# ODD2/DFD-CLIP

Hardware: AMD Instinct MI355X
Metric: 1-sec clips/sec (30x224x224 frames) ViT-B/16 (higher is better)
Workload: dtype bf16

## Files before the change

dfd-clip_amd/capi.py:

```python
import ctypes
import os
from ctypes import POINTER, Structure, c_char_p, c_double, c_float, c_int, c_int32, c_int64, c_size_t, c_uint32, c_void_p

import torch

PKG_DIR = os.path.dirname(os.path.abspath(__file__))
LIB_PATH = os.path.join(PKG_DIR, "libdfdclip_hip.so")

F32, BF16 = 0, 1
EPI_BIAS, EPI_BIAS_QUICKGELU, EPI_BIAS_RESIDUAL, EPI_PATCH_EMBED, EPI_QKV_EXPORT, EPI_RESIDUAL_POS, EPI_BIAS_GELU = range(7)
ABI_VERSION = 17

_DTYPE = {torch.float32: F32, torch.bfloat16: BF16}
FP8 = 2
FP8_MAX = 448.0
FP8_MIN_ROWS = 1024


class DfdError(RuntimeError):
    pass


GEMM_STREAM_OUT = 1
GEMM_SPARE_IF_FREE = 2
GEMM_C_BLOCKED = 4
GEMM_A_BLOCKED = 8


class GemmExtra(Structure):
    _fields_ = [("pos", c_void_p), ("cls", c_void_p), ("k_export", c_void_p), ("v_export", c_void_p),
                ("tokens", c_int32), ("frames_per_clip", c_int32), ("residual", c_void_p), ("qkv_first", c_int32),
                ("drop_rng", c_void_p), ("drop_site", c_uint32), ("drop_p", c_float), ("flags", c_uint32)]


OPTIM_SGD, OPTIM_ADAMW = 0, 1


class OptimExtra(Structure):
    _fields_ = [("kind", c_int32), ("reserved", c_int32), ("beta1", c_double), ("beta2", c_double), ("eps", c_double),
                ("step", c_int64), ("exp_avg_sq", c_void_p)]


class DropoutDesc(Structure):
    _fields_ = [("rng_state", c_void_p), ("site", c_uint32), ("p", c_float)]


class Dropout:
    __slots__ = ("rng", "site", "p")

    def __init__(self, rng, site, p):
        assert rng.is_cuda and rng.dtype == torch.int64 and rng.numel() == 2 and 0.0 <= p < 1.0
        self.rng, self.site, self.p = rng, int(site), float(p)

    def desc(self):
        return DropoutDesc(self.rng.data_ptr(), self.site, self.p)


def _drop(d):
    return ctypes.byref(d.desc()) if d is not None and d.p > 0 else None
# ... 227 lines not shown
    s3 = (c_float * 3)(*[float(v) for v in std])
    if patch_rows:
        assert out.dim() == 2 and out.shape[0] == n * (res // patch) ** 2
        kpad = out.shape[1]
    else:
        assert tuple(out.shape) == (n, 3, res, res)
        kpad = 0
    _check(load_library().dfd_preprocess_u8(_ptr(frames), n, h, w, res, patch, int(bool(antialias)), m3, s3, _ptr(out),
                                            _DTYPE[out.dtype], 1 if patch_rows else 0, kpad, _stream()), "dfd_preprocess_u8")
    return out


_profile = {"epilogue": None, "events": [], "base": None}


def profile_gemm(epilogue=None):
    _profile["epilogue"] = epilogue
    _profile["events"] = []
    _profile["base"] = None
    if epilogue is not None:
        _profile["base"] = torch.cuda.Event(enable_timing=True)
        _profile["base"].record()


def profile_gemm_collect():
    base = _profile["base"]
    spans = [(base.elapsed_time(a), base.elapsed_time(b), flops) for a, b, flops in _profile["events"]]
    profile_gemm(None)
    return spans


def gemm(a, w, c, bias=None, epilogue=EPI_BIAS, m=None, pos=None, cls=None, k_export=None, v_export=None, tokens=0,
         frames_per_clip=0, residual=None, qkv_first=0, drop=None, stream_out=False, spare_cus=0, tile_blocks=0, spare_if_free=False,
         c_blocked=False, a_blocked=False):
    _dev(a, w, c, bias, pos, cls, k_export, v_export, residual)
    assert a.dtype == w.dtype and a.stride(1) == 1 and w.stride(1) == 1 and c.stride(1) == 1
    M = a.shape[0] if m is None else m
    N, K = w.shape
    assert a.shape[1] == K
    assert residual is None or (residual.dtype == c.dtype and residual.stride(0) == c.stride(0))
    assert drop is None or epilogue == EPI_RESIDUAL_POS
    assert 0 <= epilogue <= EPI_BIAS_GELU, f"unknown epilogue {epilogue}"
    if c_blocked or a_blocked:
        blk = c if c_blocked else a
        assert blk.shape[0] >= (M + 15) // 16 * 16, "a blocked matrix needs its rows rounded up to 16"
    extra = GemmExtra(_ptr(pos).value, _ptr(cls).value, _ptr(k_export).value, _ptr(v_export).value, tokens, frames_per_clip,
                      _ptr(residual).value, qkv_first, drop.rng.data_ptr() if drop is not None and drop.p > 0 else None,
                      drop.site if drop is not None else 0, drop.p if drop is not None else 0.0, (GEMM_STREAM_OUT if stream_out else 0) | (GEMM_SPARE_IF_FREE if spare_if_free else 0) | ((int(spare_cus) & 0xff) << 8) | ((int(tile_blocks) & 0xf) << 16)
                      | (GEMM_C_BLOCKED if c_blocked else 0) | (GEMM_A_BLOCKED if a_blocked else 0))
    timed = _profile["epilogue"] == epilogue
    if timed:
        e0, e1 = torch.cuda.Event(enable_timing=True), torch.cuda.Event(enable_timing=True)
        e0.record()
    _check(load_library().dfd_gemm(_ptr(a), a.stride(0), _ptr(w), w.stride(0), _DTYPE[a.dtype], _ptr(c), c.stride(0),
                                   _DTYPE[c.dtype], _ptr(bias), epilogue, ctypes.byref(extra), M, N, K, _stream()), "dfd_gemm")
    if timed:
        e1.record()
        _profile["events"].append((e0, e1, 2.0 * M * N * K))
    return c


def gemm_fp8(a, w, c, col_scale, bias=None, epilogue=EPI_BIAS, m=None, out_inv_scale=0.0, pos=None, k_export=None, v_export=None,
             tokens=0, frames_per_clip=0, qkv_first=0, stream_out=False, spare_cus=0, spare_if_free=False):
    _dev(a, w, c, col_scale, bias, pos, k_export, v_export)
    assert a.element_size() == 1 and w.element_size() == 1 and a.stride(1) == 1 and w.stride(1) == 1 and c.stride(1) == 1
    assert col_scale.dtype == torch.float32 and col_scale.is_contiguous()
    M = a.shape[0] if m is None else m
    N, K = w.shape
    assert a.shape[1] == K and col_scale.numel() == N
    c_dtype = FP8 if c.element_size() == 1 else _DTYPE[c.dtype]
    extra = GemmExtra(_ptr(pos).value, None, _ptr(k_export).value, _ptr(v_export).value, tokens, frames_per_clip, None, qkv_first,
                      None, 0, 0.0, (GEMM_STREAM_OUT if stream_out else 0) | (GEMM_SPARE_IF_FREE if spare_if_free else 0) | ((int(spare_cus) & 0xff) << 8))
    timed = _profile["epilogue"] == epilogue
    if timed:
        e0, e1 = torch.cuda.Event(enable_timing=True), torch.cuda.Event(enable_timing=True)
        e0.record()
    _check(load_library().dfd_gemm_fp8(_ptr(a), a.stride(0), _ptr(w), w.stride(0), _ptr(c), c.stride(0), c_dtype, _ptr(col_scale),
                                       _ptr(bias), float(out_inv_scale), epilogue, ctypes.byref(extra), M, N, K, _stream()),
           "dfd_gemm_fp8")
    if timed:
        e1.record()
        _profile["events"].append((e0, e1, 2.0 * M * N * K))
# ... 383 lines not shown
```

dfd-clip_amd/csrc/gemm.hip:

```cpp
#include "gemm_args.hpp"
#include "gelu.hpp"
#include "../../include/dfdclip_hooks.h"

namespace {

constexpr int BM = 128, BN = 128;
constexpr int ROW_BYTES = 64;
constexpr int ROW_STRIDE = 80;
constexpr int TILE_BYTES = BM * ROW_STRIDE;
constexpr int EPI_SPLITK_SLAB = 100;

template <typename CT> __device__ __forceinline__ void store_c(void* C, int64_t off, float v) {
  static_cast<CT*>(C)[off] = from_f32<CT>(v);
}

template <typename CT, int EPI>
__device__ __forceinline__ void epilogue_elem(const GemmArgs& a, int64_t m, int n, float acc) {
  if (m >= a.M || n >= a.N) return;
  if constexpr (EPI == DFD_EPI_BIAS) {
    store_c<CT>(a.C, m * a.ldc + n, acc + (a.bias ? a.bias[n] : 0.f));
  } else if constexpr (EPI == DFD_EPI_BIAS_QUICKGELU) {
    store_c<CT>(a.C, m * a.ldc + n, quick_gelu(acc + (a.bias ? a.bias[n] : 0.f)));
  } else if constexpr (EPI == DFD_EPI_BIAS_GELU) {
    store_c<CT>(a.C, m * a.ldc + n, gelu_erf(acc + (a.bias ? a.bias[n] : 0.f)));
// ... 237 lines not shown
}

static int fill_extra(GemmArgs& a, int epilogue, const dfd_gemm_extra* extra, int c_dtype, int64_t ldc, int64_t M, int N) {
  if (epilogue == DFD_EPI_PATCH_EMBED) {
    DFD_REQUIRE(extra && extra->pos && extra->cls && extra->tokens > 1, "dfd_gemm: PATCH_EMBED needs extra.pos, extra.cls, extra.tokens");
    DFD_REQUIRE(M % (extra->tokens - 1) == 0, "dfd_gemm: PATCH_EMBED M=%lld is not a whole number of frames", (long long)M);
    DFD_REQUIRE(c_dtype == DFD_F32 && ldc >= N, "dfd_gemm: PATCH_EMBED writes an f32 token matrix");
  } else {
    DFD_REQUIRE(ldc >= N, "dfd_gemm: ldc=%lld < N", (long long)ldc);
  }
  if (epilogue == DFD_EPI_QKV_EXPORT) {
    DFD_REQUIRE(extra && extra->tokens > 1 && (extra->qkv_first == 0 || extra->qkv_first == 1) && N % (3 - extra->qkv_first) == 0,
                "dfd_gemm: QKV_EXPORT needs extra.tokens, qkv_first in {0, 1} and N a multiple of the column blocks present");
    DFD_REQUIRE(M % extra->tokens == 0, "dfd_gemm: QKV_EXPORT M=%lld is not a whole number of frames", (long long)M);
    DFD_REQUIRE(!extra->k_export == !extra->v_export, "dfd_gemm: QKV_EXPORT needs both k_export and v_export or neither");
    DFD_REQUIRE(!extra->pos || extra->frames_per_clip > 0, "dfd_gemm: QKV_EXPORT with pos needs frames_per_clip");
  }
  if (epilogue == DFD_EPI_RESIDUAL_POS) {
    DFD_REQUIRE(extra && extra->tokens > 1, "dfd_gemm: RESIDUAL_POS needs extra.tokens (patches per frame + 1)");
    DFD_REQUIRE(!extra->pos || extra->frames_per_clip > 0, "dfd_gemm: RESIDUAL_POS with pos needs frames_per_clip");
  }
  if (extra) {
    a.pos = extra->pos; a.cls = extra->cls; a.k_export = extra->k_export; a.v_export = extra->v_export;
    a.residual = epilogue == DFD_EPI_RESIDUAL_POS ? extra->residual : nullptr;
    a.tokens = extra->tokens; a.frames_per_clip = extra->frames_per_clip > 0 ? extra->frames_per_clip : 1;
    a.qkv_first = epilogue == DFD_EPI_QKV_EXPORT ? extra->qkv_first : 0;
    a.stream_out = (extra->flags & DFD_GEMM_STREAM_OUT) ? 1 : 0;
    a.spare_cus = (int)((extra->flags >> DFD_GEMM_SPARE_CUS_SHIFT) & 0xff);
    a.spare_if_free = (extra->flags & DFD_GEMM_SPARE_IF_FREE) ? 1 : 0;
    a.tile_rows = 32 * (int)((extra->flags >> DFD_GEMM_TILE_BLOCKS_SHIFT) & 0xf);
    a.c_blocked = (extra->flags & DFD_GEMM_C_BLOCKED) ? 1 : 0;
    a.a_blocked = (extra->flags & DFD_GEMM_A_BLOCKED) ? 1 : 0;
    a.pair = a.c_blocked | a.a_blocked;
    DFD_REQUIRE(a.tile_rows == 0 || a.tile_rows == 224 || a.tile_rows == 256, "dfd_gemm: tile blocks must be 0, 7 or 8");
    if (epilogue == DFD_EPI_RESIDUAL_POS && extra->drop_rng && extra->drop_p > 0.f) {
      DFD_REQUIRE(extra->drop_p < 1.f, "dfd_gemm: drop_p=%f", (double)extra->drop_p);
      const dfd_dropout_t dd{extra->drop_rng, extra->drop_site, extra->drop_p};
      a.drop = dfd_make_drop(&dd);
    }
  }
  return DFD_OK;
}

static thread_local int g_last_path = 0;
static thread_local int g_gemm_variant = 0;
extern "C" int dfd_gemm_last_path(void) { return g_last_path; }
extern "C" int dfd_gemm_set_variant(int variant) {
  const int old = g_gemm_variant;
  g_gemm_variant = variant;
  return old;
}

static thread_local int g_pair_variant = 0;
static thread_local int64_t g_pair_launches = 0;
extern "C" int dfd_gemm_pair_set_variant(int variant) {
  const int old = g_pair_variant;
  g_pair_variant = variant;
  return old;
}
extern "C" int64_t dfd_gemm_pair_launches(void) { return g_pair_launches; }
extern "C" int dfd_gemm_pair_plan(int64_t M, int D, int H) {
  if (g_pair_variant == 1 || g_gemm_variant == 1 || M < 1 || D < 1 || H < 1) return 0;
  if (M < 1024 && g_pair_variant != 2) return 0;
  void* const any = reinterpret_cast<void*>(uintptr_t{256});
  GemmArgs fc{}, pr{};
  fc.A = pr.A = any; fc.W = pr.W = any; fc.C = pr.C = any;
  fc.M = pr.M = M; fc.pair = pr.pair = 1;
  fc.N = H; fc.K = D; fc.lda = D; fc.ldw = D; fc.ldc = H; fc.c_blocked = 1;
  pr.N = D; pr.K = H; pr.lda = H; pr.ldw = H; pr.ldc = D; pr.a_blocked = 1;
  return dfd_gemm256e_serves(fc, DFD_BF16, DFD_EPI_BIAS_QUICKGELU) && dfd_gemm256e_serves(pr, DFD_BF16, DFD_EPI_BIAS) ? 1 : 0;
}

static int try_persistent_kernels(GemmArgs& a, int c_dtype, int epilogue, bool f8, hipStream_t st, int* path) {
  const int epi_p = epilogue == DFD_EPI_QKV_EXPORT && a.k_export == nullptr ? DFD_EPI_BIAS : epilogue;
  a.no_dynamic = g_gemm_variant != 3;
  if (a.pair) {
    if (g_pair_variant == 1) a.c_blocked = a.a_blocked = 0;
    *path = 257;
    const int rc = f8 || g_gemm_variant == 1 ? 1 : dfd_gemm256e_try(a, c_dtype, epi_p, st);
    if (rc == 1) {
      dfd_set_error("dfd_gemm: DFD_GEMM_C_BLOCKED / DFD_GEMM_A_BLOCKED: the ping-pong kernel does not serve this call (bf16, N %% 256 == 0, "
                    "K %% 128 == 0, K >= 384, ld %% 64 == 0, BIAS_QUICKGELU / BIAS_GELU for C, BIAS for A; got M=%lld N=%d K=%d)",
                    (long long)a.M, a.N, a.K);
      return DFD_ERR_INVALID_ARG;
    }
    if (rc == 0 && (a.c_blocked || a.a_blocked)) ++g_pair_launches;
    return rc;
  }
  int rc = g_gemm_variant == 1 ? 1 : (f8 ? dfd_gemm256e_f8_try : dfd_gemm256e_try)(a, c_dtype, epi_p, st);
  *path = 257;
  if (rc != 1) return rc;
  rc = (f8 ? dfd_gemm256p_f8_try : dfd_gemm256p_try)(a, c_dtype, epi_p, st);
  *path = 256;
  return rc;
}

extern "C" int dfd_gemm(const void* A, int64_t lda, const void* W, int64_t ldw, int ab_dtype, void* C, int64_t ldc,
                        int c_dtype, const float* bias, int epilogue, const dfd_gemm_extra* extra, int64_t M, int N,
                        int K, void* stream) {
  DFD_REQUIRE(A && W && C, "dfd_gemm: null pointer");
  DFD_REQUIRE(M >= 0 && N > 0 && K > 0, "dfd_gemm: bad shape M=%lld N=%d K=%d", (long long)M, N, K);
  DFD_REQUIRE(ab_dtype == DFD_F32 || ab_dtype == DFD_BF16, "dfd_gemm: ab_dtype=%d", ab_dtype);
  DFD_REQUIRE(c_dtype == DFD_F32 || c_dtype == DFD_BF16, "dfd_gemm: c_dtype=%d", c_dtype);
  DFD_REQUIRE(!(ab_dtype == DFD_F32 && c_dtype == DFD_BF16), "dfd_gemm: f32 operands with bf16 output unsupported");
  DFD_REQUIRE(K % 32 == 0, "dfd_gemm: K=%d must be a multiple of 32", K);
  const int esz = ab_dtype == DFD_F32 ? 4 : 2;
  DFD_REQUIRE(lda >= K && ldw >= K && (lda * esz) % 16 == 0 && (ldw * esz) % 16 == 0, "dfd_gemm: lda=%lld ldw=%lld must be >= K and 16-byte multiples", (long long)lda, (long long)ldw);
  DFD_REQUIRE(dfd_aligned16(A) && dfd_aligned16(W), "dfd_gemm: A and W must be 16-byte aligned");
// ... 81 lines not shown
```

dfd-clip_amd/csrc/gemm256e.hip:

```cpp
#include <mutex>
#include <unordered_map>

#include "gemm256p_common.hpp"

namespace {

constexpr int UNIT = 128 * ROWB;
constexpr int DEPTH = 6;
constexpr int NB = 2 * (DEPTH - 1);

template <int EPI, int RB, bool F8, bool CF8, bool ABLK = false>
__global__ __launch_bounds__(512) void gemm256e_kernel(const GemmArgs a, int tiles_m, int tiles_n) {
  static_assert(!F8 || RB == 8, "fp8 form: 256-row tiles only");
  static_assert(!CF8 || (F8 && EPI != DFD_EPI_QKV_EXPORT), "fp8 output: fp8 operands, plain, QuickGELU or GELU epilogue");
  constexpr int ESZ = F8 ? 1 : 2;
  constexpr int TMU = 32 * RB;
  constexpr int WROWS = 16 * RB;
  constexpr int HB = RB - 4;
  constexpr int NCV = F8 ? 2 : 1;
  constexpr int S1 = CF8 ? RB : 2 * RB;
  constexpr int S2 = 4 * RB;
  static_assert(!ABLK || (!F8 && EPI == DFD_EPI_BIAS), "blocked A: bf16 operands, plain epilogue");
  constexpr bool C_BLK = !F8 && (EPI == DFD_EPI_BIAS_QUICKGELU || EPI == DFD_EPI_BIAS_GELU);
  constexpr bool A_BLK = ABLK;
  __shared__ __attribute__((aligned(1024))) unsigned char smem[RING + 8 * STAGE];
  const int tid = threadIdx.x;
  const int lane = tid & 63;
  const int wave = __builtin_amdgcn_readfirstlane(tid >> 6);
  const int wr = wave >> 2, wc = wave & 3;
  const int ntiles = tiles_m * tiles_n;

  const int G = gridDim.x, bid = blockIdx.x;
  const int xcd = bid & 7, q8 = G >> 3, r8 = G & 7;
  const int pos = xcd_position();

  const OperandSrds<F8, CF8, A_BLK, C_BLK> srd(a);
  const __amdgpu_buffer_rsrc_t srdA = srd.A, srdW = srd.W, srdC = srd.C;
  const v4i srdB = words(a.bias ? a.bias : reinterpret_cast<const float*>(a.W), a.bias ? a.N * 4 : 0);
  [[maybe_unused]] const v4i srdS = words(F8 ? a.col_scale : reinterpret_cast<const float*>(a.W), F8 ? a.N * 4 : 0);
  const int cnt_x = q8 + (xcd < r8 ? 1 : 0), off_x = pos - (bid >> 3);
  const v4i srdT = words(reinterpret_cast<const float*>(a.sched ? a.sched : reinterpret_cast<const uint32_t*>(a.W)), a.sched ? 8 * 128 : 0);

  const uint32_t lda2 = (uint32_t)(a.lda * ESZ), ldw2 = (uint32_t)(a.ldw * ESZ);
  const uint32_t a_last = (uint32_t)(a.M - 1) * lda2;
  constexpr bool a_blk = A_BLK;
  constexpr int a_kstep = a_blk ? (int)DFD_BLK_UNIT : ROWB;
  uint32_t vA[2][2], vW[2];
  auto set_a = [&](const Tile& t, int ha) {
    int l = lane;
    asm volatile("" : "+v"(l));
    const uint32_t pr = (uint32_t)(l >> 3), pp = (uint32_t)(l & 7);
    if constexpr (a_blk) {
      const uint32_t c0 = pp ^ (pr >> 1);
// ... 298 lines not shown
    if (pool == nullptr) {
      if (hipMalloc(reinterpret_cast<void**>(&pool), MAX_SLOTS * 8 * 128) != hipSuccess || hipMemset(pool, 0, MAX_SLOTS * 8 * 128) != hipSuccess) {
        (void)hipGetLastError();
        pool = nullptr;
        return true;
      }
    }
    if (used >= MAX_SLOTS) return true;
    SchedSlot sl;
    sl.dev = pool + used * 8 * 32;
    ++used;
    it = slots.emplace(st, sl).first;
  }
  SchedSlot& sl = it->second;
  a.sched = sl.dev;
  const int q8 = grid >> 3, r8 = grid & 7;
  const int64_t full = ntiles / grid, rem = ntiles % grid;
  for (int x = 0; x < 8; ++x) {
    a.sched_base[x] = sl.base[x];
    const int cnt = q8 + (x < r8 ? 1 : 0);
    const int off = x < r8 ? x * (q8 + 1) : r8 * (q8 + 1) + (x - r8) * q8;
    int64_t last = rem - off;
    last = last < 0 ? 0 : (last > cnt ? cnt : last);
    sl.base[x] += (uint32_t)(full * cnt + last);
  }
  return true;
}

struct Gemm256e {
  static constexpr const char* name = "ping-pong";
  static constexpr bool spare_if_free = true;
  static constexpr bool blocked_layout = true;
  static constexpr bool serves(int epi, bool f8) {
    return epi == DFD_EPI_BIAS || epi == DFD_EPI_BIAS_QUICKGELU || epi == DFD_EPI_BIAS_GELU || epi == DFD_EPI_QKV_EXPORT || (!f8 && epi == DFD_EPI_RESIDUAL_POS);
  }
  static bool depth_ok(const GemmArgs& a, int esz, int nk, int epi) {
    if ((nk < 6 && !(epi == DFD_EPI_RESIDUAL_POS && nk == 4)) || (nk & 1)) return false;
    return (a.ldw * esz) % 128 == 0;
  }
  static void prepare(GemmArgs& a, hipStream_t st, const TilePlan& p, bool f8) {
    if (!f8 && a.K / TK >= 6 && a.no_dynamic == 0) sched_prepare(a, st, p.grid, p.ntiles);
    else a.sched = nullptr;
  }
  template <int EPI, int RB, bool F8, bool CF8>
  static void run(int grid, hipStream_t st, const GemmArgs& a, int tiles_m, int tiles_n) {
    if constexpr (!F8 && EPI == DFD_EPI_BIAS) {
      if (a.a_blocked) {
        hipLaunchKernelGGL((gemm256e_kernel<EPI, RB, F8, CF8, true>), dim3(grid), dim3(512), 0, st, a, tiles_m, tiles_n);
        return;
      }
    }
    hipLaunchKernelGGL((gemm256e_kernel<EPI, RB, F8, CF8, false>), dim3(grid), dim3(512), 0, st, a, tiles_m, tiles_n);
  }
};

}

int dfd_gemm256e_try(const GemmArgs& a, int c_dtype, int epi, hipStream_t st) { return try_persistent<Gemm256e, false>(a, c_dtype, epi, st); }

int dfd_gemm256e_serves(const GemmArgs& a, int c_dtype, int epi) { return persistent_serves<Gemm256e, false>(a, c_dtype, epi) == 0; }

int dfd_gemm256e_f8_try(const GemmArgs& a, int c_dtype, int epi, hipStream_t st) { return try_persistent<Gemm256e, true>(a, c_dtype, epi, st); }
```

dfd-clip_amd/csrc/gemm256p_common.hpp:

```cpp
#pragma once
#include <type_traits>

#include "gemm_args.hpp"

#include "gelu.hpp"
#include "gemm_blocked.hpp"

typedef int v4i_t __attribute__((ext_vector_type(4)));
typedef v4i_t v4i;
typedef int v8i __attribute__((ext_vector_type(8)));

inline int persistent_cu_count() {
  static int n_cu = 0;
  if (n_cu == 0) {
    int dev = 0;
    hipDeviceProp_t prop;
    if (hipGetDevice(&dev) == hipSuccess && hipGetDeviceProperties(&prop, dev) == hipSuccess) n_cu = prop.multiProcessorCount;
  }
  return n_cu;
}

namespace {

__device__ __forceinline__ void store_out(v4i_t d, __amdgpu_buffer_rsrc_t srd, uint32_t off, int stream_out) {
// ... 43 lines not shown

__device__ __forceinline__ __amdgpu_buffer_rsrc_t make_srd(const void* p, int64_t bytes) {
  return __builtin_amdgcn_make_buffer_rsrc(const_cast<void*>(p), 0, (int)(uint32_t)bytes, 0x00020000);
}
__device__ __forceinline__ v4i words(const float* p, int bytes) {
  const uint64_t u = reinterpret_cast<uint64_t>(p);
  return v4i{(int)(uint32_t)u, (int)((uint32_t)(u >> 32) & 0xffffu), bytes, 0x00020000};
}
template <bool F8, bool CF8, bool ABLK = false, bool CBLK = false>
struct OperandSrds {
  __amdgpu_buffer_rsrc_t A, W, C;
  __device__ __forceinline__ explicit OperandSrds(const GemmArgs& a)
      : A(make_srd(a.A, rows(a.M, ABLK && a.a_blocked) * a.lda * (F8 ? 1 : 2))), W(make_srd(a.W, (int64_t)a.N * a.ldw * (F8 ? 1 : 2))),
        C(make_srd(a.C, rows(a.M, CBLK && a.c_blocked) * a.ldc * (CF8 ? 1 : 2))) {}
  static __device__ __forceinline__ int64_t rows(int64_t M, bool blocked) { return blocked ? (M + 15) & ~(int64_t)15 : M; }
};
template <int RB> __device__ __forceinline__ int countable_stores(int stores, const Tile& t, int wr, int64_t M) {
  return (int64_t)t.m0 + (wr + 1) * 16 * RB <= M ? stores : 0;
}

template <int EPI, int RB, bool F8, bool CF8, bool BLK = false>
__device__ __forceinline__ int tile_epilogue(const GemmArgs& a, f32x4 (&acc)[RB][4], const f32x4 (&b4)[4], const f32x4 (&cs4)[4], unsigned char* const ep,
                                             const Tile& cur, int wr, int wc, int le, int D, __amdgpu_buffer_rsrc_t srdC) {
  constexpr int WROWS = 16 * RB;
  const int er = le & 15, eq = le >> 4;
  const int drow = le >> 3, dc = le & 7;
  const int nb = cur.n0 + wc * 64;
  const int64_t mrow0 = (int64_t)cur.m0 + wr * WROWS + drow;
  const int rows_left = (int)min((int64_t)0x7fffffff, a.M - mrow0);
  int which = 0;
  if constexpr (EPI == DFD_EPI_QKV_EXPORT) which = cur.n0 / D + a.qkv_first;
  const bool exporting = EPI == DFD_EPI_QKV_EXPORT && which > 0 && a.k_export != nullptr;
  int stores = 2 * RB;
#pragma unroll
  for (int i = 0; i < RB; ++i)
#pragma unroll
    for (int j = 0; j < 4; ++j) {
      if constexpr (F8) acc[i][j] = acc[i][j] * cs4[j] + b4[j];
      else acc[i][j] += b4[j];
    }
  if constexpr (EPI == DFD_EPI_QKV_EXPORT) {
    if (exporting) {
      stores = 4 * RB;
      const int ecol = nb - (which - a.qkv_first) * D + dc * 8;
      unsigned char* const parkf = ep + er * 256;
      const int64_t erows = (a.M / a.tokens) * (a.tokens - 1);
      const __amdgpu_buffer_rsrc_t srdE = make_srd(which == 2 ? a.v_export : a.k_export, erows * D * 2);
      const __amdgpu_buffer_rsrc_t srdP = make_srd(a.pos ? a.pos : reinterpret_cast<const float*>(a.W), a.pos ? a.frames_per_clip * D * 4 : 0);
#pragma unroll
      for (int i = 0; i < RB; ++i) {
        __builtin_amdgcn_sched_barrier(0);
        uint32_t eoff[2];
        f32x4 pe[2][2];
#pragma unroll
        for (int rr = 0; rr < 2; ++rr) {
          const int rloc = i * 16 + rr * 8;
          const uint32_t m = (uint32_t)min(mrow0 + rloc, a.M - 1);
          const uint32_t frame = a.div_tokens.div(m);
          const uint32_t tok = m - frame * (uint32_t)a.tokens;
          const uint32_t t = frame - a.div_frames.div(frame) * (uint32_t)a.frames_per_clip;
          eoff[rr] = (rloc < rows_left && tok > 0) ? ((frame * (uint32_t)(a.tokens - 1) + tok - 1) * (uint32_t)D + ecol) * 2 : 0xffffffffu;
          pe[rr][0] = pe[rr][1] = f32x4{0.f, 0.f, 0.f, 0.f};
          if (a.pos != nullptr) {
            const uint32_t poff = (t * (uint32_t)D + ecol) * 4;
            pe[rr][0] = __builtin_bit_cast(f32x4, __builtin_amdgcn_raw_buffer_load_b128(srdP, poff, 0, 0));
            pe[rr][1] = __builtin_bit_cast(f32x4, __builtin_amdgcn_raw_buffer_load_b128(srdP, poff, 16, 0));
          }
        }
#pragma unroll
        for (int j = 0; j < 4; ++j)
          *reinterpret_cast<f32x4*>(parkf + (((j * 4 + eq) ^ er) << 4)) = acc[i][j];
#pragma unroll
        for (int rr = 0; rr < 2; ++rr) {
// ... 62 lines not shown
    for (int i = 0; i < RB; ++i) {
      __builtin_amdgcn_sched_barrier(0);
      const int b = i & 1;
      if (i + 1 < RB) request(i + 1, b ^ 1);
#pragma unroll
      for (int j = 0; j < 4; ++j) *reinterpret_cast<f32x4*>(parkf + (((j * 4 + eq) ^ er) << 4)) = acc[i][j];
      if (i == 0) wait_vm<6>();
      else if (i + 1 < RB) wait_vm<8>();
      else wait_vm<2>();
      asm volatile("" : "+v"(pq[b][0][0]), "+v"(pq[b][0][1]), "+v"(oq[b][0]), "+v"(pq[b][1][0]), "+v"(pq[b][1][1]), "+v"(oq[b][1]));
      __builtin_amdgcn_sched_barrier(0);
#pragma unroll
      for (int rr = 0; rr < 2; ++rr) {
        const int row = rr * 8 + drow;
        const f32x4 x0 = *reinterpret_cast<const f32x4*>(ep + row * 256 + (((2 * dc) ^ row) << 4));
        const f32x4 x1 = *reinterpret_cast<const f32x4*>(ep + row * 256 + (((2 * dc + 1) ^ row) << 4));
        float dv[8];
#pragma unroll
        for (int e = 0; e < 4; ++e) {
          dv[e] = x0[e];
          dv[4 + e] = x1[e];
        }
        dfd_drop_eight(a.drop, (uint64_t)gq[b][rr] << 3, dv);
        const bf16x8 ob = __builtin_bit_cast(bf16x8, oq[b][rr]);
        bf16x8 o;
#pragma unroll
        for (int e = 0; e < 4; ++e) {
          o[e] = (bf16_t)((float)ob[e] + dv[e] + pq[b][rr][0][e]);
          o[4 + e] = (bf16_t)((float)ob[4 + e] + dv[4 + e] + pq[b][rr][1][e]);
        }
        store_out(__builtin_bit_cast(v4i, o), srdC, offq[b][rr], a.stream_out);
      }
    }
  } else if constexpr (CF8) {
    stores = RB;
    const int srow = le >> 2, sc = le & 3;
    unsigned char* const park8 = ep + er * 64 + eq * 4;
    const int psw = (er >> 1) & 3;
    const unsigned char* const dsrc8 = ep + srow * 64 + ((sc ^ ((srow >> 1) & 3)) << 4);
    const int64_t m8 = (int64_t)cur.m0 + wr * WROWS + srow;
    const int rows_left8 = (int)min((int64_t)0x7fffffff, a.M - m8);
    const uint32_t cbase8 = (uint32_t)(m8 * a.ldc + nb + sc * 16);
#pragma unroll
    for (int q = 0; q < 4; ++q) {
#pragma unroll
      for (int ii = 0; ii < 2; ++ii) {
        const int i = 2 * q + ii;
#pragma unroll
        for (int j = 0; j < 4; ++j) {
          f32x4 v = activate(acc[i][j]) * a.out_inv_scale;
#pragma unroll
          for (int e = 0; e < 4; ++e) v[e] = __builtin_fminf(__builtin_fmaxf(v[e], -448.0f), 448.0f);
          unsigned pk = __builtin_amdgcn_cvt_pk_fp8_f32(v[0], v[1], 0u, false);
          pk = __builtin_amdgcn_cvt_pk_fp8_f32(v[2], v[3], pk, true);
          *reinterpret_cast<unsigned*>(park8 + ii * 1024 + ((j ^ psw) << 4)) = pk;
        }
      }
#pragma unroll
      for (int rr = 0; rr < 2; ++rr) {
        const v4i d = *reinterpret_cast<const v4i*>(dsrc8 + rr * 1024);
        const int rloc = q * 32 + rr * 16;
        const uint32_t off = rloc < rows_left8 ? cbase8 + (uint32_t)rloc * (uint32_t)a.ldc : 0xffffffffu;
        store_out(d, srdC, off, a.stream_out);
      }
    }
  } else if (BLK && a.c_blocked) {
// ... 97 lines not shown
    return DFD_ERR_LAUNCH;
  }
  return DFD_OK;
}

inline int check_persistent(const GemmArgs& a, int esz, int csz, int kstep) {
  if (a.N % TN != 0 || a.K % kstep != 0 || (a.M < 1024 && !a.pair)) return 1;
  if ((a.lda * esz) % 16 != 0 || (a.ldw * esz) % 16 != 0 || (a.ldc * csz) % 16 != 0) return 1;
  if ((reinterpret_cast<uintptr_t>(a.A) & 15) != 0 || (reinterpret_cast<uintptr_t>(a.W) & 15) != 0 || (reinterpret_cast<uintptr_t>(a.C) & 15) != 0) return 1;
  if (a.bias && (reinterpret_cast<uintptr_t>(a.bias) & 15) != 0) return 1;
  const int64_t lim = (int64_t)0xfffffff0;
  const int64_t Mr = a.pair ? (a.M + 15) & ~(int64_t)15 : a.M;
  if (Mr * a.lda * esz > lim || (int64_t)a.N * a.ldw * esz > lim || Mr * a.ldc * csz > lim) return 1;
  if ((int64_t)((a.M + 223) / 224) * (a.N / TN) > 0x3fffffff || a.M >= ((int64_t)1 << 31)) return 1;
  if ((a.c_blocked || a.a_blocked) && (esz != 2 || csz != 2)) return 1;
  if ((a.c_blocked && a.ldc % 64 != 0) || (a.a_blocked && a.lda % 64 != 0)) return 1;
  return 0;
}

inline int check_export(const GemmArgs& a) {
  if ((a.N / (3 - a.qkv_first)) % TN != 0) return 1;
  if (a.pos && (reinterpret_cast<uintptr_t>(a.pos) & 15) != 0) return 1;
  if (a.k_export && (a.M / a.tokens) * (a.tokens - 1) * (int64_t)(a.N / (3 - a.qkv_first)) * 2 > (int64_t)0xfffffff0) return 1;
  return 0;
}

inline int check_residual_pos(const GemmArgs& a) {
  if (a.tokens < 2 || a.M * (int64_t)(a.N >> 3) >= ((int64_t)1 << 32)) return 1;
  if (a.pos && ((reinterpret_cast<uintptr_t>(a.pos) & 15) != 0 || a.frames_per_clip < 1)) return 1;
  if (a.residual && (reinterpret_cast<uintptr_t>(a.residual) & 15) != 0) return 1;
  return 0;
}

template <class L, bool F8>
int persistent_serves(const GemmArgs& a_in, int c_dtype, int epi) {
  if (c_dtype != DFD_BF16 && !(F8 && c_dtype == DFD_FP8)) return 1;
  const bool cf8 = c_dtype == DFD_FP8;
  constexpr int esz = F8 ? 1 : 2, kstep = F8 ? 128 : TK;
  if (F8 && (!a_in.col_scale || (reinterpret_cast<uintptr_t>(a_in.col_scale) & 15) != 0)) return 1;
  if (check_persistent(a_in, esz, cf8 ? 1 : 2, kstep) || !L::depth_ok(a_in, esz, a_in.K / kstep, epi)) return 1;
  if (!L::serves(epi, F8)) return 1;
  if ((a_in.c_blocked || a_in.a_blocked) && !L::blocked_layout) return 1;
  if (a_in.c_blocked && epi != DFD_EPI_BIAS_QUICKGELU && epi != DFD_EPI_BIAS_GELU) return 1;
  if (a_in.a_blocked && epi != DFD_EPI_BIAS) return 1;
  return 0;
}

template <class L, bool F8>
int try_persistent(const GemmArgs& a_in, int c_dtype, int epi, hipStream_t st) {
  if (persistent_serves<L, F8>(a_in, c_dtype, epi)) return 1;
  const bool cf8 = c_dtype == DFD_FP8;
  GemmArgs a = a_in;
  auto go = [&](auto epi_c) -> int {
    constexpr int EPI = decltype(epi_c)::value;
    constexpr bool rows_to_frames = EPI == DFD_EPI_QKV_EXPORT || EPI == DFD_EPI_RESIDUAL_POS;
    if constexpr (!L::serves(EPI, F8)) {
      return 1;
    } else {
      if constexpr (EPI == DFD_EPI_QKV_EXPORT) {
        if (check_export(a)) return 1;
      }
      if constexpr (EPI == DFD_EPI_RESIDUAL_POS) {
        if (check_residual_pos(a)) return 1;
      }
      if constexpr (rows_to_frames) {
        a.div_tokens = FastDiv::make((uint32_t)(EPI == DFD_EPI_RESIDUAL_POS ? a.tokens - 1 : a.tokens));
        a.div_frames = FastDiv::make((uint32_t)(a.frames_per_clip > 0 ? a.frames_per_clip : 1));
      }
      if constexpr (F8 && !rows_to_frames) {
        if (cf8) return launch_persistent<L, EPI, true, true>(a, st);
      }
      return cf8 ? 1 : launch_persistent<L, EPI, F8, false>(a, st);
    }
  };
  switch (epi) {
    case DFD_EPI_BIAS:
      return go(std::integral_constant<int, DFD_EPI_BIAS>{});
    case DFD_EPI_BIAS_QUICKGELU:
      return go(std::integral_constant<int, DFD_EPI_BIAS_QUICKGELU>{});
    case DFD_EPI_BIAS_GELU:
      return go(std::integral_constant<int, DFD_EPI_BIAS_GELU>{});
    case DFD_EPI_QKV_EXPORT:
      return go(std::integral_constant<int, DFD_EPI_QKV_EXPORT>{});
    case DFD_EPI_RESIDUAL_POS:
      return go(std::integral_constant<int, DFD_EPI_RESIDUAL_POS>{});
    default:
      return 1;
  }
}

}
```

dfd-clip_amd/csrc/gemm_args.hpp:

```cpp
#pragma once
#include "dropout.hpp"

struct GemmArgs {
  const void* A;
  const void* W;
  void* C;
  const float* bias;
  const float* pos;
  const float* cls;
  void* k_export;
  void* v_export;
  const void* residual;
  int64_t lda, ldw, ldc, M;
  int N, K, tokens, frames_per_clip;
  int qkv_first;
  int stream_out;
  int spare_cus;
  int spare_if_free;
  int tile_rows;
  DfdDrop drop;
  FastDiv div_tokens, div_frames;
  const float* col_scale;
  float out_inv_scale;
  uint32_t* sched;
  uint32_t sched_base[8];
  int no_dynamic;
  int c_blocked, a_blocked, pair;
};

int dfd_gemm256_try(const GemmArgs& a, int c_dtype, int epi, hipStream_t st);
int dfd_gemm256e_try(const GemmArgs& a, int c_dtype, int epi, hipStream_t st);
int dfd_gemm256e_serves(const GemmArgs& a, int c_dtype, int epi);
int dfd_gemm256e_f8_try(const GemmArgs& a, int c_dtype, int epi, hipStream_t st);
int dfd_gemm256p_try(const GemmArgs& a, int c_dtype, int epi, hipStream_t st);
int dfd_gemm256p_f8_try(const GemmArgs& a, int c_dtype, int epi, hipStream_t st);
```

dfd-clip_amd/encoder.py:

```python
import contextlib

import torch
from torch import nn

from . import blocked, capi


FP8_PRESETS = ("all", "proj-bf16", "kv-bf16", "kv+proj-bf16", "edges-bf16", "none")
FP8_CONTRACT_POLICY = None
_ALL = {"qkv": "fp8", "fc": "fp8", "proj": "fp8"}
_NONE = {"qkv": "bf16", "fc": "bf16", "proj": "bf16"}


def expand_fp8_policy(policy, layers, tapped=None):
    tapped = sorted(set(range(layers) if tapped is None else (int(t) for t in tapped)))
    if any(t < 0 or t >= layers for t in tapped):
        raise ValueError(f"fp8 policy: tapped layers {tapped} outside 0..{layers - 1}")
    if policy is None:
        policy = "all"
    if isinstance(policy, str):
        if policy not in FP8_PRESETS:
            raise ValueError(f"fp8 policy: unknown preset {policy!r} (presets: {', '.join(FP8_PRESETS)})")
        kv = "kv-bf16" if policy in ("kv-bf16", "kv+proj-bf16") else "fp8"
        proj = "bf16" if policy in ("proj-bf16", "kv+proj-bf16") else "fp8"
# ... 304 lines not shown
                patches=torch.zeros(Pp, kpad, device=dev, dtype=act),
                delta=torch.zeros(Mp, D, device=dev, dtype=act) if self.deferred_residual else None,
                delta2=torch.zeros(Mp, D, device=dev, dtype=act) if self.deferred_residual else None, pending=0,
                qkv=[torch.zeros(Mp, 3 * D, device=dev, dtype=act) for _ in range(keep_layers)])
            if need_h8:
                ws["h8"] = torch.zeros(Mp, D, device=dev, dtype=torch.uint8)
            if need_u8:
                ws["u8"] = torch.zeros(Mp, 4 * D, device=dev, dtype=torch.uint8)
            if len(self._ws) > 6:
                self._ws.clear()
            self._ws[key] = ws
        return ws

    def graph_guard(self, n):
        return (self._prepare(), self._fp8_layers() if self.precision == "fp8" else None, self._workspace(n, 1, slot=0))

    def _as_frames(self, x):
        if x.dtype == torch.uint8:
            assert x.dim() == 4 and x.shape[1] == 3, "uint8 frames must be [N, 3, H, W]"
            return x.contiguous()
        assert tuple(x.shape[1:]) == (3, self.input_resolution, self.input_resolution), \
            f"frames must be [N, 3, {self.input_resolution}, {self.input_resolution}]"
        return x.to(torch.float32).contiguous()

    def _embed(self, frames, ws, p):
        n = frames.shape[0]
        P, D = self.tokens - 1, self.width
        if frames.dtype == torch.uint8:
            capi.preprocess_u8(frames, ws["patches"][:n * P], self.input_resolution, self.patch_size, self.pixel_mean,
                               self.pixel_std, antialias=self.antialias)
        else:
            capi.patchify(frames, ws["patches"], self.input_resolution, self.patch_size)
        capi.gemm(ws["patches"], p["w_patch"], ws["x"], None, capi.EPI_PATCH_EMBED, m=n * P, pos=p["pos"], cls=p["cls"],
                  tokens=self.tokens)
        ws["pending"] = 0
        ws["ln_pre"] = p["ln_pre"]

    def _ln(self, ws, gb, M, store=True, q=None, discard_x=False, dual=False):
        x = ws["x"]
        if dual:
            return self._ln_dual(ws, gb, M, q, discard_x)
        h, inv = (ws["h8"], q) if q is not None else (ws["h"], 0.0)
        pend = ws.get("pending", 0)
        pre = ws.pop("ln_pre", None)
        if pre is not None:
            assert pend == 0
            if self.width <= 2048:
                capi.layernorm2(x[:M], pre[0], pre[1], gb[0], gb[1], h[:M], eps=self.ln_eps, out_inv_scale=inv)
            else:
                capi.layernorm(x[:M], pre[0], pre[1], x[:M], eps=self.ln_eps)
                capi.layernorm(x[:M], gb[0], gb[1], h[:M], eps=self.ln_eps, out_inv_scale=inv)
        elif pend == 0:
            capi.layernorm(x[:M], gb[0], gb[1], h[:M], eps=self.ln_eps, out_inv_scale=inv)
        elif discard_x:
            capi.add_layernorm(x[:M], ws["delta"][:M], gb[0], gb[1], h[:M], delta2=ws["delta2"][:M] if pend == 2 else None,
                               store_x=False, eps=self.ln_eps, out_inv_scale=inv)
            ws["pending"] = 0
        elif not store:
            assert pend == 1
            capi.add_layernorm(x[:M], ws["delta"][:M], gb[0], gb[1], h[:M], store_x=False, eps=self.ln_eps, out_inv_scale=inv)
        else:
            capi.add_layernorm(x[:M], ws["delta"][:M], gb[0], gb[1], h[:M], delta2=ws["delta2"][:M] if pend == 2 else None,
                               eps=self.ln_eps, out_inv_scale=inv)
            ws["pending"] = 0

    def _ln_dual(self, ws, gb, M, inv, discard_x):
        x, h, h8 = ws["x"], ws["h"], ws["h8"]
# ... 179 lines not shown
```

include/dfdclip.h:

```cpp
#ifndef DFDCLIP_H
#define DFDCLIP_H

#include <stddef.h>
#include <stdint.h>

#ifdef __cplusplus
extern "C" {
#endif

#define DFD_ABI_VERSION 17

enum { DFD_F32 = 0, DFD_BF16 = 1, DFD_FP8 = 2  };

enum {
  DFD_OK = 0,
  DFD_ERR_INVALID_ARG = -1,
  DFD_ERR_LAUNCH = -2,
  DFD_ERR_NO_DEVICE = -3
};

enum {
  DFD_EPI_BIAS = 0,
  DFD_EPI_BIAS_QUICKGELU,
  DFD_EPI_BIAS_RESIDUAL,
  DFD_EPI_PATCH_EMBED,
  DFD_EPI_QKV_EXPORT,
  DFD_EPI_RESIDUAL_POS,
  DFD_EPI_BIAS_GELU
};

typedef struct dfd_dropout_t {
  const uint64_t* rng_state;
  uint32_t site;
  float p;
} dfd_dropout_t;

typedef struct dfd_gemm_extra {
  const float* pos;
  const float* cls;
  void* k_export;
  void* v_export;
  int32_t tokens;
  int32_t frames_per_clip;
  const void* residual;
  int32_t qkv_first;
  const uint64_t* drop_rng;
  uint32_t drop_site;
  float drop_p;
  uint32_t flags;
} dfd_gemm_extra;

enum {
  DFD_GEMM_STREAM_OUT = 1,
  DFD_GEMM_SPARE_IF_FREE = 2,
  DFD_GEMM_C_BLOCKED = 4,
  DFD_GEMM_A_BLOCKED = 8,
  DFD_GEMM_TILE_BLOCKS_SHIFT = 16,
  DFD_GEMM_SPARE_CUS_SHIFT = 8
};

const char* dfd_last_error(void);
int dfd_abi_version(void);
int dfd_device_check(void);

int dfd_layernorm(const float* x, int64_t ldx, const float* gamma, const float* beta, void* y, int64_t ldy,
                  int y_dtype, int64_t rows, int cols, float eps, float y_inv_scale, void* stream);

int dfd_layernorm2(float* x, int64_t ldx, const float* gamma_a, const float* beta_a, const float* gamma_b, const float* beta_b,
                   void* y, int64_t ldy, int y_dtype, int64_t rows, int cols, float eps, float y_inv_scale, void* stream);

int dfd_add_layernorm(float* x, int64_t ldx, const void* delta, const void* delta2, int64_t ldd, int delta_dtype,
                      int store_x, const float* gamma, const float* beta, void* y, int64_t ldy, int y_dtype, int64_t rows,
                      int cols, float eps, float y_inv_scale, void* stream);


int dfd_patchify(const float* frames, void* patches, int out_dtype, int n_frames, int res, int patch, int kpad,
                 void* stream);

int dfd_preprocess_u8(const uint8_t* frames, int n_frames, int in_h, int in_w, int res, int patch, int antialias,
                      const float* mean3, const float* std3, void* out, int out_dtype, int layout, int kpad,
                      void* stream);
int dfd_preprocess_geometry(int in_h, int in_w, int res, int* rs_h, int* rs_w, int* top, int* left);

int dfd_gemm(const void* A, int64_t lda, const void* W, int64_t ldw, int ab_dtype, void* C, int64_t ldc,
             int c_dtype, const float* bias, int epilogue, const dfd_gemm_extra* extra, int64_t M, int N, int K,
             void* stream);
int dfd_gemm_fp8(const void* A, int64_t lda, const void* W, int64_t ldw, void* C, int64_t ldc, int c_dtype,
                 const float* col_scale, const float* bias, float out_inv_scale, int epilogue,
                 const dfd_gemm_extra* extra, int64_t M, int N, int K, void* stream);
// ... 120 lines not shown
```

Before: 877.6.

## Route patch-embed GEMM through persistent 256 kernel with fused pos/cls epilogue

Adds a PATCH_EMBED epilogue to the persistent 256-tile GEMM. It writes f32 tokens into the frame layout, adds positional embeddings loaded via buffer loads, and writes cls+pos rows. It is enabled by a new flag that the encoder now sets for the patch projection, so that GEMM leaves the older generic kernel path. The goal is a faster patch-embedding GEMM, at the cost of extra per-row division and pos loads in the epilogue. Other callers still bypass the persistent path for patch embed.

```diff
diff --git a/dfd-clip_amd/capi.py b/dfd-clip_amd/capi.py
--- a/dfd-clip_amd/capi.py
+++ b/dfd-clip_amd/capi.py
@@ -25,6 +25,7 @@
 GEMM_SPARE_IF_FREE = 2
 GEMM_C_BLOCKED = 4
 GEMM_A_BLOCKED = 8
+GEMM_PATCH_PERSISTENT = 16
 
 
 class GemmExtra(Structure):
@@ -318,7 +319,7 @@
 
 def gemm(a, w, c, bias=None, epilogue=EPI_BIAS, m=None, pos=None, cls=None, k_export=None, v_export=None, tokens=0,
          frames_per_clip=0, residual=None, qkv_first=0, drop=None, stream_out=False, spare_cus=0, tile_blocks=0, spare_if_free=False,
-         c_blocked=False, a_blocked=False):
+         c_blocked=False, a_blocked=False, patch_persistent=False):
     _dev(a, w, c, bias, pos, cls, k_export, v_export, residual)
     assert a.dtype == w.dtype and a.stride(1) == 1 and w.stride(1) == 1 and c.stride(1) == 1
     M = a.shape[0] if m is None else m
@@ -333,7 +334,8 @@
     extra = GemmExtra(_ptr(pos).value, _ptr(cls).value, _ptr(k_export).value, _ptr(v_export).value, tokens, frames_per_clip,
                       _ptr(residual).value, qkv_first, drop.rng.data_ptr() if drop is not None and drop.p > 0 else None,
                       drop.site if drop is not None else 0, drop.p if drop is not None else 0.0, (GEMM_STREAM_OUT if stream_out else 0) | (GEMM_SPARE_IF_FREE if spare_if_free else 0) | ((int(spare_cus) & 0xff) << 8) | ((int(tile_blocks) & 0xf) << 16)
-                      | (GEMM_C_BLOCKED if c_blocked else 0) | (GEMM_A_BLOCKED if a_blocked else 0))
+                      | (GEMM_C_BLOCKED if c_blocked else 0) | (GEMM_A_BLOCKED if a_blocked else 0)
+                      | (GEMM_PATCH_PERSISTENT if patch_persistent else 0))
     timed = _profile["epilogue"] == epilogue
     if timed:
         e0, e1 = torch.cuda.Event(enable_timing=True), torch.cuda.Event(enable_timing=True)
diff --git a/dfd-clip_amd/csrc/gemm.hip b/dfd-clip_amd/csrc/gemm.hip
--- a/dfd-clip_amd/csrc/gemm.hip
+++ b/dfd-clip_amd/csrc/gemm.hip
@@ -293,6 +293,7 @@
     a.c_blocked = (extra->flags & DFD_GEMM_C_BLOCKED) ? 1 : 0;
     a.a_blocked = (extra->flags & DFD_GEMM_A_BLOCKED) ? 1 : 0;
     a.pair = a.c_blocked | a.a_blocked;
+    a.patch_persistent = (extra->flags & DFD_GEMM_PATCH_PERSISTENT) ? 1 : 0;
     DFD_REQUIRE(a.tile_rows == 0 || a.tile_rows == 224 || a.tile_rows == 256, "dfd_gemm: tile blocks must be 0, 7 or 8");
     if (epilogue == DFD_EPI_RESIDUAL_POS && extra->drop_rng && extra->drop_p > 0.f) {
       DFD_REQUIRE(extra->drop_p < 1.f, "dfd_gemm: drop_p=%f", (double)extra->drop_p);
@@ -335,6 +336,7 @@
 static int try_persistent_kernels(GemmArgs& a, int c_dtype, int epilogue, bool f8, hipStream_t st, int* path) {
   const int epi_p = epilogue == DFD_EPI_QKV_EXPORT && a.k_export == nullptr ? DFD_EPI_BIAS : epilogue;
   a.no_dynamic = g_gemm_variant != 3;
+  if (epilogue == DFD_EPI_PATCH_EMBED && (!a.patch_persistent || f8)) return 1;
   if (a.pair) {
     if (g_pair_variant == 1) a.c_blocked = a.a_blocked = 0;
     *path = 257;
diff --git a/dfd-clip_amd/csrc/gemm256e.hip b/dfd-clip_amd/csrc/gemm256e.hip
--- a/dfd-clip_amd/csrc/gemm256e.hip
+++ b/dfd-clip_amd/csrc/gemm256e.hip
@@ -18,7 +18,7 @@
   constexpr int WROWS = 16 * RB;
   constexpr int HB = RB - 4;
   constexpr int NCV = F8 ? 2 : 1;
-  constexpr int S1 = CF8 ? RB : 2 * RB;
+  constexpr int S1 = CF8 ? RB : EPI == DFD_EPI_PATCH_EMBED ? 5 * RB : 2 * RB;
   constexpr int S2 = 4 * RB;
   static_assert(!ABLK || (!F8 && EPI == DFD_EPI_BIAS), "blocked A: bf16 operands, plain epilogue");
   constexpr bool C_BLK = !F8 && (EPI == DFD_EPI_BIAS_QUICKGELU || EPI == DFD_EPI_BIAS_GELU);
@@ -383,7 +383,8 @@
   static constexpr bool spare_if_free = true;
   static constexpr bool blocked_layout = true;
   static constexpr bool serves(int epi, bool f8) {
-    return epi == DFD_EPI_BIAS || epi == DFD_EPI_BIAS_QUICKGELU || epi == DFD_EPI_BIAS_GELU || epi == DFD_EPI_QKV_EXPORT || (!f8 && epi == DFD_EPI_RESIDUAL_POS);
+    return epi == DFD_EPI_BIAS || epi == DFD_EPI_BIAS_QUICKGELU || epi == DFD_EPI_BIAS_GELU || epi == DFD_EPI_QKV_EXPORT ||
+           (!f8 && (epi == DFD_EPI_RESIDUAL_POS || epi == DFD_EPI_PATCH_EMBED));
   }
   static bool depth_ok(const GemmArgs& a, int esz, int nk, int epi) {
     if ((nk < 6 && !(epi == DFD_EPI_RESIDUAL_POS && nk == 4)) || (nk & 1)) return false;
diff --git a/dfd-clip_amd/csrc/gemm256p_common.hpp b/dfd-clip_amd/csrc/gemm256p_common.hpp
--- a/dfd-clip_amd/csrc/gemm256p_common.hpp
+++ b/dfd-clip_amd/csrc/gemm256p_common.hpp
@@ -99,13 +99,15 @@
   if constexpr (EPI == DFD_EPI_QKV_EXPORT) which = cur.n0 / D + a.qkv_first;
   const bool exporting = EPI == DFD_EPI_QKV_EXPORT && which > 0 && a.k_export != nullptr;
   int stores = 2 * RB;
-#pragma unroll
-  for (int i = 0; i < RB; ++i)
-#pragma unroll
-    for (int j = 0; j < 4; ++j) {
-      if constexpr (F8) acc[i][j] = acc[i][j] * cs4[j] + b4[j];
-      else acc[i][j] += b4[j];
-    }
+  if constexpr (EPI != DFD_EPI_PATCH_EMBED) {
+#pragma unroll
+    for (int i = 0; i < RB; ++i)
+#pragma unroll
+      for (int j = 0; j < 4; ++j) {
+        if constexpr (F8) acc[i][j] = acc[i][j] * cs4[j] + b4[j];
+        else acc[i][j] += b4[j];
+      }
+  }
   if constexpr (EPI == DFD_EPI_QKV_EXPORT) {
     if (exporting) {
       stores = 4 * RB;
@@ -234,6 +236,80 @@
         store_out(__builtin_bit_cast(v4i, o), srdC, offq[b][rr], a.stream_out);
       }
     }
+  } else if constexpr (EPI == DFD_EPI_PATCH_EMBED) {
+    stores = 5 * RB;
+    unsigned char* const parkf = ep + er * 256;
+    const int srow = le >> 4, sc = le & 15;
+    const uint32_t P = (uint32_t)(a.tokens - 1);
+    const uint32_t ldc4 = (uint32_t)(a.ldc * 4);
+    const uint32_t col4 = (uint32_t)(nb + sc * 4) * 4;
+    const int64_t mw0 = (int64_t)cur.m0 + wr * WROWS;
+    const int rows_left4 = (int)min((int64_t)0x7fffffff, a.M - (mw0 + srow));
+    const uint32_t m_last = (uint32_t)(a.M - 1);
+    const __amdgpu_buffer_rsrc_t srdX = make_srd(a.C, (int64_t)(a.M / P) * a.tokens * a.ldc * 4);
+    const v4i srdQw = words(a.pos, (int)(uint32_t)((int64_t)a.tokens * a.N * 4));
+    f32x4 clsv;
+    {
+      const v4i srdLw = words(a.cls, a.N * 4);
+      f32x4 p0;
+      asm volatile(
+          "s_nop 4\n\t"
+          "buffer_load_dwordx4 %0, %2, %3, 0 offen\n\t"
+          "buffer_load_dwordx4 %1, %2, %4, 0 offen"
+          : "=&v"(clsv), "=&v"(p0)
+          : "v"(col4), "s"(srdLw), "s"(srdQw)
+          : "memory");
+      f32x4 pq[2][4];
+      uint32_t offx[2][4];
+      auto request = [&](int i, int b) {
+        uint32_t poff[4];
+#pragma unroll
+        for (int r = 0; r < 4; ++r) {
+          const int rloc = i * 16 + r * 4;
+          const uint32_t m = min((uint32_t)(mw0 + srow + rloc), m_last);
+          const uint32_t frame = a.div_tokens.div(m);
+          const uint32_t tok = m - frame * P + 1u;
+          offx[b][r] = rloc < rows_left4 ? (frame * (uint32_t)a.tokens + tok) * ldc4 + col4 : 0xffffffffu;
+          poff[r] = tok * (uint32_t)(a.N * 4) + col4;
+        }
+        asm volatile(
+            "s_nop 4\n\t"
+            "buffer_load_dwordx4 %0, %4, %8, 0 offen\n\t"
+            "buffer_load_dwordx4 %1, %5, %8, 0 offen\n\t"
+            "buffer_load_dwordx4 %2, %6, %8, 0 offen\n\t"
+            "buffer_load_dwordx4 %3, %7, %8, 0 offen"
+            : "=&v"(pq[b][0]), "=&v"(pq[b][1]), "=&v"(pq[b][2]), "=&v"(pq[b][3])
+            : "v"(poff[0]), "v"(poff[1]), "v"(poff[2]), "v"(poff[3]), "s"(srdQw)
+            : "memory");
+      };
+      request(0, 0);
+#pragma unroll
+      for (int i = 0; i < RB; ++i) {
+        __builtin_amdgcn_sched_barrier(0);
+        const int b = i & 1;
+        if (i + 1 < RB) request(i + 1, b ^ 1);
+#pragma unroll
+        for (int j = 0; j < 4; ++j) *reinterpret_cast<f32x4*>(parkf + (((j * 4 + eq) ^ er) << 4)) = acc[i][j];
+        if (i == 0) wait_vm<4>();
+        else if (i + 1 < RB) wait_vm<9>();
+        else wait_vm<5>();
+        asm volatile("" : "+v"(pq[b][0]), "+v"(pq[b][1]), "+v"(pq[b][2]), "+v"(pq[b][3]));
+        if (i == 0) {
+          asm volatile("" : "+v"(clsv), "+v"(p0));
+          clsv = clsv + p0;
+        }
+        __builtin_amdgcn_sched_barrier(0);
+#pragma unroll
+        for (int r = 0; r < 4; ++r) {
+          const int row = r * 4 + srow;
+          const f32x4 x = *reinterpret_cast<const f32x4*>(ep + row * 256 + ((sc ^ row) << 4)) + pq[b][r];
+          store_out(__builtin_bit_cast(v4i, x), srdX, offx[b][r], a.stream_out);
+        }
+        const uint32_t fc = a.div_tokens.div(min((uint32_t)(mw0 + i * 16 + 15), m_last));
+        const uint32_t offc = srow == 0 ? fc * (uint32_t)a.tokens * ldc4 + col4 : 0xffffffffu;
+        store_out(__builtin_bit_cast(v4i, clsv), srdX, offc, a.stream_out);
+      }
+    }
   } else if constexpr (CF8) {
     stores = RB;
     const int srow = le >> 2, sc = le & 3;
@@ -397,13 +473,22 @@
   return 0;
 }
 
+inline int check_patch_embed(const GemmArgs& a) {
+  if (a.tokens < 17 || !a.pos || !a.cls || a.M % (a.tokens - 1) != 0) return 1;
+  if ((reinterpret_cast<uintptr_t>(a.pos) & 15) != 0 || (reinterpret_cast<uintptr_t>(a.cls) & 15) != 0) return 1;
+  const int64_t lim = (int64_t)0xfffffff0;
+  if ((a.M / (a.tokens - 1)) * a.tokens * a.ldc * 4 > lim || (int64_t)a.tokens * a.N * 4 > lim) return 1;
+  return 0;
+}
+
 template <class L, bool F8>
 int persistent_serves(const GemmArgs& a_in, int c_dtype, int epi) {
-  if (c_dtype != DFD_BF16 && !(F8 && c_dtype == DFD_FP8)) return 1;
+  const bool cf32 = !F8 && epi == DFD_EPI_PATCH_EMBED;
+  if (cf32 ? c_dtype != DFD_F32 : (c_dtype != DFD_BF16 && !(F8 && c_dtype == DFD_FP8))) return 1;
   const bool cf8 = c_dtype == DFD_FP8;
   constexpr int esz = F8 ? 1 : 2, kstep = F8 ? 128 : TK;
   if (F8 && (!a_in.col_scale || (reinterpret_cast<uintptr_t>(a_in.col_scale) & 15) != 0)) return 1;
-  if (check_persistent(a_in, esz, cf8 ? 1 : 2, kstep) || !L::depth_ok(a_in, esz, a_in.K / kstep, epi)) return 1;
+  if (check_persistent(a_in, esz, cf32 ? 4 : cf8 ? 1 : 2, kstep) || !L::depth_ok(a_in, esz, a_in.K / kstep, epi)) return 1;
   if (!L::serves(epi, F8)) return 1;
   if ((a_in.c_blocked || a_in.a_blocked) && !L::blocked_layout) return 1;
   if (a_in.c_blocked && epi != DFD_EPI_BIAS_QUICKGELU && epi != DFD_EPI_BIAS_GELU) return 1;
@@ -418,7 +503,7 @@
   GemmArgs a = a_in;
   auto go = [&](auto epi_c) -> int {
     constexpr int EPI = decltype(epi_c)::value;
-    constexpr bool rows_to_frames = EPI == DFD_EPI_QKV_EXPORT || EPI == DFD_EPI_RESIDUAL_POS;
+    constexpr bool rows_to_frames = EPI == DFD_EPI_QKV_EXPORT || EPI == DFD_EPI_RESIDUAL_POS || EPI == DFD_EPI_PATCH_EMBED;
     if constexpr (!L::serves(EPI, F8)) {
       return 1;
     } else {
@@ -428,8 +513,11 @@
       if constexpr (EPI == DFD_EPI_RESIDUAL_POS) {
         if (check_residual_pos(a)) return 1;
       }
+      if constexpr (EPI == DFD_EPI_PATCH_EMBED) {
+        if (check_patch_embed(a)) return 1;
+      }
       if constexpr (rows_to_frames) {
-        a.div_tokens = FastDiv::make((uint32_t)(EPI == DFD_EPI_RESIDUAL_POS ? a.tokens - 1 : a.tokens));
+        a.div_tokens = FastDiv::make((uint32_t)(EPI == DFD_EPI_QKV_EXPORT ? a.tokens : a.tokens - 1));
         a.div_frames = FastDiv::make((uint32_t)(a.frames_per_clip > 0 ? a.frames_per_clip : 1));
       }
       if constexpr (F8 && !rows_to_frames) {
@@ -449,6 +537,8 @@
       return go(std::integral_constant<int, DFD_EPI_QKV_EXPORT>{});
     case DFD_EPI_RESIDUAL_POS:
       return go(std::integral_constant<int, DFD_EPI_RESIDUAL_POS>{});
+    case DFD_EPI_PATCH_EMBED:
+      return go(std::integral_constant<int, DFD_EPI_PATCH_EMBED>{});
     default:
       return 1;
   }
diff --git a/dfd-clip_amd/csrc/gemm_args.hpp b/dfd-clip_amd/csrc/gemm_args.hpp
--- a/dfd-clip_amd/csrc/gemm_args.hpp
+++ b/dfd-clip_amd/csrc/gemm_args.hpp
@@ -26,6 +26,7 @@
   uint32_t sched_base[8];
   int no_dynamic;
   int c_blocked, a_blocked, pair;
+  int patch_persistent;
 };
 
 int dfd_gemm256_try(const GemmArgs& a, int c_dtype, int epi, hipStream_t st);
diff --git a/dfd-clip_amd/encoder.py b/dfd-clip_amd/encoder.py
--- a/dfd-clip_amd/encoder.py
+++ b/dfd-clip_amd/encoder.py
@@ -360,7 +360,7 @@
         else:
             capi.patchify(frames, ws["patches"], self.input_resolution, self.patch_size)
         capi.gemm(ws["patches"], p["w_patch"], ws["x"], None, capi.EPI_PATCH_EMBED, m=n * P, pos=p["pos"], cls=p["cls"],
-                  tokens=self.tokens)
+                  tokens=self.tokens, patch_persistent=True)
         ws["pending"] = 0
         ws["ln_pre"] = p["ln_pre"]
 
diff --git a/include/dfdclip.h b/include/dfdclip.h
--- a/include/dfdclip.h
+++ b/include/dfdclip.h
@@ -55,6 +55,7 @@
   DFD_GEMM_SPARE_IF_FREE = 2,
   DFD_GEMM_C_BLOCKED = 4,
   DFD_GEMM_A_BLOCKED = 8,
+  DFD_GEMM_PATCH_PERSISTENT = 16,
   DFD_GEMM_TILE_BLOCKS_SHIFT = 16,
   DFD_GEMM_SPARE_CUS_SHIFT = 8
 };
```

After: 876.9, median of 2. No clear change (-0.1%).
